# c0gent/hbbft

Measured on AMD Instinct MI355X. Metric: verified BLS sig shares/sec (whole node) + combine latency, N=64 f=21, higher is better.
Workload: dtype u32 limbs (Fp, 14x28-bit); 1 GPU; ThresholdSign share verification, BASELINE configs[1]; batch_per_gpu=65536, streams=2, documents_per_gpu=1024, n_nodes=64, f=21, pairing_impl=auto, parallelism=shard-by-batch x1

## Files before the change

hbbft_amd/csrc/k_pair.hip:

```cpp
#define HS_MULFN static __device__ __noinline__
#include "pair_side.hpp"

namespace hbs {

constexpr int EXP_TOP = 57;
constexpr uint64_t EXP_HIGH = hb::X_ABS >> EXP_TOP;
constexpr int EXP_HIGH_BITS = 64 - EXP_TOP;
constexpr int EXP_NPARK = __builtin_popcountll(hb::X_ABS) - __builtin_popcountll(EXP_HIGH) + 1;
static_assert((hb::X_ABS & 1) == 0 && (hb::X_ABS >> 63) == 1 && (EXP_HIGH & 1) == 1 && EXP_NPARK >= 1,
              "the base is no factor of f^|x|, and the power at bit EXP_TOP is the last one parked");
struct ExpPark {
  int32_t c[EXP_NPARK][4][NL];
  int32_t base[6][NL];
  int32_t pre[EXP_NPARK][NL];
};

HP_D void park_fp(int32_t (&d)[NL], const Fp& a) {
#pragma unroll
  for (int i = 0; i < NL; i++) d[i] = a.l[i];
}
HP_D Fp unpark_fp(const int32_t (&s)[NL]) {
  Fp r;
#pragma unroll
  for (int i = 0; i < NL; i++) r.l[i] = s[i];
  return r;
}
HP_D H12 unpark12(const int32_t (&s)[6][NL]) {
  return {{unpark_fp(s[0]), unpark_fp(s[1]), unpark_fp(s[2])}, {unpark_fp(s[3]), unpark_fp(s[4]), unpark_fp(s[5])}};
}

static __device__ __noinline__ void h_exp_gs(const ExpPark& pk, bool plus1, H12& out) {
  const uint64_t e = hb::X_ABS + (plus1 ? 1 : 0);
  H12 r = unpark12(pk.base);
#pragma unroll 1
  for (int k = 62; k >= 0; k--) {
    r = h12_cyclo_sqr(r);
    if ((e >> k) & 1) r = h12_mul<LanePair>(r, unpark12(pk.base));
  }
  out = r;
}

HP_D H12 h_exp_high(const H12& t) {
  H12 r = t;
#pragma unroll 1
  for (int k = EXP_HIGH_BITS - 2; k >= 0; k--) {
    r = h12_cyclo_sqr(r);
    if ((EXP_HIGH >> k) & 1) r = h12_mul<LanePair>(r, t);
  }
  return r;
}

static __device__ __noinline__ bool h_exp_tail(ExpPark& pk, bool plus1, H12& out) {
  Fp P;
#pragma unroll 1
  for (int j = 0; j < EXP_NPARK; j++) {
    const Fp d = hc_denom(unpark_fp(pk.c[j][0]));
    if (j == 0) P = d; else P = h_mul(P, d);
    park_fp(pk.pre[j], P);
  }
  if (h_is_zero(P)) return false;
  Fp I = fp_reduce(h_inv_vartime(P));
  H12 acc;
#pragma unroll 1
  for (int j = EXP_NPARK - 1; j >= (plus1 ? -1 : 0); j--) {
    H12 E;
    if (j >= 0) {
      const HC c = {unpark_fp(pk.c[j][0]), unpark_fp(pk.c[j][1]), unpark_fp(pk.c[j][2]), unpark_fp(pk.c[j][3])};
      Fp di = I;
      if (j > 0) {
        di = h_mul(I, unpark_fp(pk.pre[j - 1]));
        I = h_mul(I, hc_denom(c.a1));
      }
      E = hc_decompress(c, di);
    } else {
      E = unpark12(pk.base);
    }
    if (j == EXP_NPARK - 1) acc = h_exp_high(E); else acc = h12_mul<LanePair>(acc, E);
  }
  out = acc;
  return true;
}

template <bool PLUS1>
HP_D H12 h_exp_abs_x(const H12& base, ExpPark& pk) {
  park_fp(pk.base[0], base.c0.c0); park_fp(pk.base[1], base.c0.c1); park_fp(pk.base[2], base.c0.c2);
  park_fp(pk.base[3], base.c1.c0); park_fp(pk.base[4], base.c1.c1); park_fp(pk.base[5], base.c1.c2);
  HC c = hc_compress(base);
  int slot = 0;
#pragma unroll 1
  for (int k = 1; k <= EXP_TOP; k++) {
    c = hc_sqr(c);
    if ((hb::X_ABS >> k) & 1) {
      park_fp(pk.c[slot][0], c.a1); park_fp(pk.c[slot][1], c.a2);
      park_fp(pk.c[slot][2], c.a4); park_fp(pk.c[slot][3], c.a5);
      slot++;
    }
  }
  H12 r;
  if (!h_exp_tail(pk, PLUS1, r)) h_exp_gs(pk, PLUS1, r);
  return r;
}
struct ExpCompressed {
  ExpPark pk;
  HP_D H12 x(const H12& f) { return h12_conj(h_exp_abs_x<false>(f, pk)); }
  HP_D H12 xm1(const H12& f) { return h12_conj(h_exp_abs_x<true>(f, pk)); }
};

template <bool W1, bool W2, int GEN>
__global__ void __launch_bounds__(256, 2) k_pair_verify(PairArgs a) {
  extern __shared__ uint32_t stash_lds[];
  lane_verify<LanePair, ExpCompressed, W1, W2, GEN>(a, stash_lds);
}

}

namespace hbl {

struct PairKernels {
  static constexpr int LANES = hbs::LanePair::LANES;
  template <bool W1, bool W2, int GEN>
  static constexpr auto kernel = hbs::k_pair_verify<W1, W2, GEN>;
};

size_t pair_table_bytes(size_t nq) { return nq * (size_t)hbs::PAIR_STEPS * hbs::LINE_Q4 * 16; }

hipError_t pair_verify(hipStream_t s, int n, const PairSideDesc& d1, const PairSideDesc& d2, int flags,
                       uint8_t* verdict, uint32_t* value_out) {
  if (n <= 0) return hipSuccess;
  const int gen = pair_gen_mode(d1, d2);
  if (gen == 1) return lane_launch<PairKernels, 1>(s, n, d1, d2, flags, verdict, value_out);
  if (gen == 2) return lane_launch<PairKernels, 2>(s, n, d1, d2, flags, verdict, value_out);
  return lane_launch<PairKernels, 0>(s, n, d1, d2, flags, verdict, value_out);
}

}
```

hbbft_amd/csrc/pfp.hpp:

```cpp
#pragma once
#include "sfp.hpp"
#include "words.hpp"

#define HP_D __device__ __forceinline__
#define HP_L __attribute__((always_inline))

namespace hbs {

constexpr int DPP_SWAP = 0xB1;
constexpr int DPP_EVEN = 0xA0;
constexpr int DPP_ODD = 0xF5;

HP_D bool lp_even() { return (threadIdx.x & 1) == 0; }
template <int CTRL>
HP_D int32_t dpp(int32_t v) {
  return __builtin_amdgcn_mov_dpp(v, CTRL, 0xF, 0xF, true);
}
template <int CTRL>
HP_D Fp dpp_fp(const Fp& a) {
  Fp r;
#pragma unroll
  for (int i = 0; i < NL; i++) r.l[i] = dpp<CTRL>(a.l[i]);
  return r;
}

HS_MULFN Fp h_mul_l(HS_P14(x), HS_P14(y)) {
  const Fp a = {{HS_L14(x)}};
  const Fp b = {{HS_L14(y)}};
  const int32_t sm = lp_even() ? -1 : 0;
  int32_t Y[NL], W[NL], Z[NL];
#pragma unroll
  for (int i = 0; i < NL; i++) {
    Y[i] = dpp<DPP_EVEN>(b.l[i]);
    W[i] = dpp<DPP_ODD>(b.l[i]);
    Z[i] = (dpp<DPP_SWAP>(a.l[i]) ^ sm) - sm;
  }
  int32_t m[NL];
  int64_t acc = 0;
  Fp r;
#pragma unroll
  for (int k = 0; k < NL; k++) {
#pragma unroll
    for (int i = 0; i <= k; i++) {
      acc += (int64_t)a.l[i] * Y[k - i];
      acc += (int64_t)Z[i] * W[k - i];
    }
#pragma unroll
    for (int i = 0; i < k; i++) acc += (int64_t)m[i] * (int32_t)P_L[k - i];
    m[k] = mont_digit(acc);
    acc += (int64_t)m[k] * (int32_t)P_L[0];
    acc >>= 28;
  }
#pragma unroll
  for (int k = NL; k < 2 * NL - 1; k++) {
#pragma unroll
    for (int i = k - NL + 1; i < NL; i++) {
      acc += (int64_t)a.l[i] * Y[k - i];
      acc += (int64_t)Z[i] * W[k - i];
      acc += (int64_t)m[i] * (int32_t)P_L[k - i];
    }
    r.l[k - NL] = (int32_t)acc & MASK28;
    acc >>= 28;
  }
  r.l[NL - 1] = (int32_t)acc;
  return r;
}

HP_D Fp h_mul(const Fp& a, const Fp& b) { return h_mul_l(HS_E14(a), HS_E14(b)); }

HP_D Fp h_sqr(const Fp& a) {
  const bool ev = lp_even();
  const Fp pa = dpp_fp<DPP_SWAP>(a);
  Fp x, y;
#pragma unroll
  for (int i = 0; i < NL; i++) {
    x.l[i] = pa.l[i] + (ev ? a.l[i] : pa.l[i]);
    y.l[i] = a.l[i] - (ev ? pa.l[i] : 0);
  }
  return fp_mul(x, y);
}

HP_D Fp h_mul_xi(const Fp& a) {
  const int32_t sm = lp_even() ? -1 : 0;
  const Fp pa = dpp_fp<DPP_SWAP>(a);
  Fp r;
#pragma unroll
  for (int i = 0; i < NL; i++) r.l[i] = a.l[i] + ((pa.l[i] ^ sm) - sm);
  fp_norm(r);
  return r;
}
HP_D Fp h_conj(const Fp& a) {
  const Fp n = fp_neg(a);
  return lp_even() ? a : n;
}
HP_D Fp h_zero() { return fp_zero(); }
HP_D Fp h_one() { return lp_even() ? fp_one() : fp_zero(); }
HP_D Fp h_const(const uint32_t (&c0)[NL], const uint32_t (&c1)[NL]) {
  Fp r;
  const bool ev = lp_even();
#pragma unroll
  for (int i = 0; i < NL; i++) r.l[i] = (int32_t)(ev ? c0[i] : c1[i]);
  return r;
}
HP_D bool lp_both(bool v) { return (v ? 1 : 0) & dpp<DPP_SWAP>(v ? 1 : 0); }
HP_D bool h_is_zero(const Fp& a) { return lp_both(fp_is_zero(a)); }
template <int MODE = 0>
HP_D Fp h_inv_vartime(const Fp& a) {
  const Fp s = fp_sqr(a);
  const Fp n = fp_add(s, dpp_fp<DPP_SWAP>(s));
  uint32_t w[12], p[12], r[12];
  fp_to_words(n, w);
  uint32_t nz = 0;
#pragma unroll
  for (int i = 0; i < 12; i++) nz |= w[i];
  if (nz == 0) return fp_zero();
#pragma unroll
  for (int i = 0; i < 12; i++) p[i] = hb::PM2_W[i];
  p[0] += 2;
  hb::words_inv_vartime<12, MODE>(w, p, r);
  return h_conj(fp_mul(a, fp_from_words(r)));
}

template <int M, int K>
HP_D Fp fp_red_mk(const Fp& t, const Fp& a) {
  const int64_t top = (int64_t)t.l[NL - 1] * M + (int64_t)K * a.l[NL - 1];
  const int32_t q = (int32_t)((top * QINV) >> 32);
  Fp r;
  int64_t acc = 0;
#pragma unroll
  for (int i = 0; i < NL - 1; i++) {
    acc += (int64_t)t.l[i] * M + (int64_t)K * a.l[i] - (int64_t)q * (int32_t)P_L[i];
    r.l[i] = (int32_t)acc & MASK28;
    acc >>= 28;
  }
  r.l[NL - 1] = (int32_t)(acc + top - (int64_t)q * (int32_t)P_L[NL - 1]);
  return r;
}
HP_D Fp fp_red_l(const Fp& t) { return fp_red_mk<1, 0>(t, t); }
HP_D Fp h_add_xi_l(const Fp& s, const Fp& t) {
  const int32_t sm = lp_even() ? -1 : 0;
  const Fp pt = dpp_fp<DPP_SWAP>(t);
  Fp r;
#pragma unroll
  for (int i = 0; i < NL; i++) r.l[i] = s.l[i] + t.l[i] + ((pt.l[i] ^ sm) - sm);
  return r;
}
HP_D Fp fp_sub2l(const Fp& a, const Fp& b, const Fp& c) {
  Fp r;
#pragma unroll
  for (int i = 0; i < NL; i++) r.l[i] = a.l[i] - b.l[i] - c.l[i];
  return r;
}

HP_D Fp h_xi_l(const Fp& t) {
  const int32_t sm = lp_even() ? -1 : 0;
  const Fp pt = dpp_fp<DPP_SWAP>(t);
  Fp r;
#pragma unroll
  for (int i = 0; i < NL; i++) r.l[i] = t.l[i] + ((pt.l[i] ^ sm) - sm);
  return r;
}

struct H6 { Fp c0, c1, c2; };
struct H12 { H6 c0, c1; };

HP_D H6 h6_zero() { return {h_zero(), h_zero(), h_zero()}; }
HP_D H6 h6_one() { return {h_one(), h_zero(), h_zero()}; }
HP_D H6 h6_add(const H6& a, const H6& b) { return {fp_add(a.c0, b.c0), fp_add(a.c1, b.c1), fp_add(a.c2, b.c2)}; }
HP_D H6 h6_sub(const H6& a, const H6& b) { return {fp_sub(a.c0, b.c0), fp_sub(a.c1, b.c1), fp_sub(a.c2, b.c2)}; }
HP_D H6 h6_neg(const H6& a) { return {fp_neg(a.c0), fp_neg(a.c1), fp_neg(a.c2)}; }
HP_D H6 h6_red(const H6& a) { return {fp_reduce(a.c0), fp_reduce(a.c1), fp_reduce(a.c2)}; }
HP_D H6 h6_mul_v(const H6& a) { return {h_mul_xi(a.c2), a.c0, a.c1}; }

HP_D H6 h6_mul(const H6& a, const H6& b) {
  const Fp v1 = h_mul(a.c1, b.c1);
  const Fp v2 = h_mul(a.c2, b.c2);
  const Fp d0 = fp_sub2l(h_mul(fp_addl(a.c1, a.c2), fp_add(b.c1, b.c2)), v1, v2);
  const Fp v0 = h_mul(a.c0, b.c0);
  const Fp c0 = fp_red_l(h_add_xi_l(v0, d0));
  const Fp c1 = fp_red_l(h_add_xi_l(fp_sub2l(h_mul(fp_addl(a.c0, a.c1), fp_add(b.c0, b.c1)), v0, v1), v2));
  const Fp c2 = fp_red_l(fp_addl(fp_sub2l(h_mul(fp_addl(a.c0, a.c2), fp_add(b.c0, b.c2)), v0, v2), v1));
  return {c0, c1, c2};
}
HP_D H6 h6_inv(const H6& a) {
  const Fp c0 = fp_reduce(fp_sub(h_sqr(a.c0), h_mul_xi(h_mul(a.c1, a.c2))));
  const Fp c1 = fp_reduce(fp_sub(h_mul_xi(h_sqr(a.c2)), h_mul(a.c0, a.c1)));
  const Fp c2 = fp_reduce(fp_sub(h_sqr(a.c1), h_mul(a.c0, a.c2)));
  const Fp t = fp_reduce(fp_add(h_mul(a.c0, c0), h_mul_xi(fp_add(h_mul(a.c2, c1), h_mul(a.c1, c2)))));
  const Fp ti = fp_reduce(h_inv_vartime(t));
  return {h_mul(c0, ti), h_mul(c1, ti), h_mul(c2, ti)};
}

HP_D H12 h12_one() { return {h6_one(), h6_zero()}; }
HP_D H12 h12_conj(const H12& a) { return {a.c0, h6_neg(a.c1)}; }
HP_D H12 h12_red(const H12& a) { return {h6_red(a.c0), h6_red(a.c1)}; }
HP_D H12 h12_kcomb(const H6& t0, const H6& t1, const H6& s) {
  return {{fp_red_l(h_add_xi_l(t0.c0, t1.c2)), fp_red_l(fp_addl(t0.c1, t1.c0)), fp_red_l(fp_addl(t0.c2, t1.c1))},
          {fp_red_l(fp_sub2l(s.c0, t0.c0, t1.c0)), fp_red_l(fp_sub2l(s.c1, t0.c1, t1.c1)),
           fp_red_l(fp_sub2l(s.c2, t0.c2, t1.c2))}};
}

HP_D H6 h6_mul_12(const H6& x, const Fp& b1, const Fp& b2) {
  const Fp u = h_mul(x.c1, b1);
  const Fp w = h_mul(x.c2, b2);
  const Fp c0 = fp_red_l(h_xi_l(fp_sub2l(h_mul(fp_addl(x.c1, x.c2), fp_add(b1, b2)), u, w)));
  const Fp c1 = fp_red_l(h_add_xi_l(h_mul(x.c0, b1), w));
  const Fp c2 = fp_red_l(fp_addl(h_mul(x.c0, b2), u));
  return {c0, c1, c2};
}

HP_D const H6& h6_of(const H6& a) { return a; }
template <class F>
HP_D auto h6_of(const F& f) -> decltype(f()) { return f(); }

template <class G>
HP_D H12 h12_mul(const H12& a, const H12& b) {
  H6 t0, t1;
  G::mul6x2(a.c0, b.c0, a.c1, b.c1, t0, t1);
  const H6 s = G::mul6(h6_add(a.c0, a.c1), h6_add(b.c0, b.c1));
  return h12_kcomb(t0, t1, s);
}
template <class G>
HP_D H12 h12_sqr(const H12& a) {
  H6 t, s;
  G::mul6x2(a.c0, a.c1, [&]() HP_L { return h6_add(a.c0, a.c1); },
            [&]() HP_L { return h6_red(h6_add(a.c0, h6_mul_v(a.c1))); }, t, s);
  return {{fp_red_l(h_add_xi_l(fp_subl(s.c0, t.c0), fp_subl(fp_zero(), t.c2))), fp_red_l(fp_sub2l(s.c1, t.c1, t.c0)),
           fp_red_l(fp_sub2l(s.c2, t.c2, t.c1))},
          {fp_red_l(fp_addl(t.c0, t.c0)), fp_red_l(fp_addl(t.c1, t.c1)), fp_red_l(fp_addl(t.c2, t.c2))}};
}
template <class G>
HP_D H12 h12_mul_lines(const H12& f, const Fp& a0, const Fp& a1, const Fp& a4, const Fp& b0, const Fp& b1,
                       const Fp& b4) {
  H6 C0, t0, t1;
  Fp c11, c12;
  G::line_product(a0, a1, a4, b0, b1, b4, C0, c11, c12);
  G::mul6x2_12(f.c0, C0, f.c1, c11, c12, t0, t1);
  const H6 s = G::mul6(h6_add(f.c0, f.c1), {C0.c0, fp_add(C0.c1, c11), fp_add(C0.c2, c12)});
  return h12_kcomb(t0, t1, s);
}
template <class G>
HP_D H12 h12_inv(const H12& a) {
  H6 s0, s1, r0, r1;
  G::mul6x2(a.c0, a.c0, a.c1, a.c1, s0, s1);
  const H6 t = h6_red(h6_sub(h6_red(s0), h6_red(h6_mul_v(h6_red(s1)))));
  const H6 ti = h6_red(h6_inv(t));
  G::mul6x2(a.c0, ti, a.c1, ti, r0, r1);
  return h12_red({r0, h6_neg(r1)});
}

#define HP_FROB1(K) h_const(hb::FROB1_##K##_C0, hb::FROB1_##K##_C1)
HP_D H12 h12_frob1(const H12& f) {
  H12 r;
  r.c0.c0 = h_conj(f.c0.c0);
  r.c1.c0 = h_mul(h_conj(f.c1.c0), HP_FROB1(1));
  r.c0.c1 = h_mul(h_conj(f.c0.c1), HP_FROB1(2));
  r.c1.c1 = h_mul(h_conj(f.c1.c1), HP_FROB1(3));
  r.c0.c2 = h_mul(h_conj(f.c0.c2), HP_FROB1(4));
  r.c1.c2 = h_mul(h_conj(f.c1.c2), HP_FROB1(5));
  return h12_red(r);
}
HP_D H12 h12_frob2(const H12& f) {
  H12 r;
  r.c0.c0 = f.c0.c0;
  r.c1.c0 = fp_mul(f.c1.c0, fp_const(hb::FROB2_1_C0));
  r.c0.c1 = fp_mul(f.c0.c1, fp_const(hb::FROB2_2_C0));
  r.c1.c1 = fp_mul(f.c1.c1, fp_const(hb::FROB2_3_C0));
  r.c0.c2 = fp_mul(f.c0.c2, fp_const(hb::FROB2_4_C0));
  r.c1.c2 = fp_mul(f.c1.c2, fp_const(hb::FROB2_5_C0));
  return r;
}

HP_D H12 h12_cyclo_sqr(const H12& f) {
  const Fp& a0 = f.c0.c0; const Fp& a2 = f.c0.c1; const Fp& a4 = f.c0.c2;
  const Fp& a1 = f.c1.c0; const Fp& a3 = f.c1.c1; const Fp& a5 = f.c1.c2;
  H12 r;
  {
    const Fp s0 = h_sqr(a0), s3 = h_sqr(a3), s03 = h_sqr(fp_add(a0, a3));
    r.c0.c0 = fp_red_mk<3, -2>(h_add_xi_l(s0, s3), a0);
    r.c1.c1 = fp_red_mk<3, 2>(fp_sub2l(s03, s0, s3), a3);
  }
  {
    const Fp s1 = h_sqr(a1), s4 = h_sqr(a4), s14 = h_sqr(fp_add(a1, a4));
    r.c0.c1 = fp_red_mk<3, -2>(h_add_xi_l(s1, s4), a2);
    r.c1.c2 = fp_red_mk<3, 2>(fp_sub2l(s14, s1, s4), a5);
  }
  {
    const Fp s2 = h_sqr(a2), s5 = h_sqr(a5), s25 = h_sqr(fp_add(a2, a5));
    r.c0.c2 = fp_red_mk<3, -2>(h_add_xi_l(s2, s5), a4);
    r.c1.c0 = fp_red_mk<3, 2>(h_add_xi_l(fp_zero(), fp_sub2l(s25, s2, s5)), a1);
  }
  return r;
}

struct HC { Fp a1, a2, a4, a5; };

HP_D HC hc_compress(const H12& f) { return {f.c1.c0, f.c0.c1, f.c0.c2, f.c1.c2}; }
HP_D HC hc_sqr(const HC& c) {
  HC r;
  {
    const Fp s1 = h_sqr(c.a1), s4 = h_sqr(c.a4), s14 = h_sqr(fp_add(c.a1, c.a4));
    r.a2 = fp_red_mk<3, -2>(h_add_xi_l(s1, s4), c.a2);
    r.a5 = fp_red_mk<3, 2>(fp_sub2l(s14, s1, s4), c.a5);
  }
  {
    const Fp s2 = h_sqr(c.a2), s5 = h_sqr(c.a5), s25 = h_sqr(fp_add(c.a2, c.a5));
    r.a4 = fp_red_mk<3, -2>(h_add_xi_l(s2, s5), c.a4);
    r.a1 = fp_red_mk<3, 2>(h_add_xi_l(fp_zero(), fp_sub2l(s25, s2, s5)), c.a1);
  }
  return r;
}
HP_D Fp hc_denom(const Fp& a1) { return fp_lin(4, a1, 0, a1); }
HP_D H12 hc_decompress(const HC& c, const Fp& di) {
  const Fp s5 = h_sqr(c.a5), s2 = h_sqr(c.a2);
  Fp t = h_xi_l(s5);
#pragma unroll
  for (int i = 0; i < NL; i++) t.l[i] += 3 * s2.l[i];
  const Fp a3 = h_mul(fp_red_mk<1, -2>(t, c.a4), di);
  const Fp u = fp_addl(fp_lin(2, h_sqr(a3), -3, h_mul(c.a4, c.a2)), h_mul(c.a1, c.a5));
  const Fp a0 = fp_red_l(h_add_xi_l(h_one(), u));
  return {{a0, c.a2, c.a4}, {c.a1, a3, c.a5}};
}

HP_D bool h12_is_one(const H12& f) {
  bool ok = fp_is_zero(fp_sub(f.c0.c0, h_one()));
  ok = ok && fp_is_zero(f.c0.c1) && fp_is_zero(f.c0.c2);
  ok = ok && fp_is_zero(f.c1.c0) && fp_is_zero(f.c1.c1) && fp_is_zero(f.c1.c2);
  return lp_both(ok);
}

struct HJac { Fp x, y, z; };
struct HLine { Fp c0, c1, c4; };

struct HProj { Fp x, y, z; };

HP_D HLine h_dbl_step_h(HProj& T) {
  const Fp C = h_sqr(T.z);
  const Fp YZ = h_sqr(fp_add(T.y, T.z));
  const Fp B = h_sqr(T.y);
  const Fp H = fp_sub(fp_sub(YZ, B), C);
  const Fp E = fp_red_mk<12, 0>(h_xi_l(C), C);
  const Fp A = h_mul(T.x, T.y);
  const Fp S = h_sqr(T.x);
  HLine l;
  l.c0 = fp_red_mk<1, -1>(B, E);
  l.c1 = fp_lin(-3, S, 0, S);
  l.c4 = H;
  const Fp Bm = fp_lin(1, B, -3, E);
  const Fp Bp = fp_lin(1, B, 3, E);
  T.x = h_mul(fp_addl(A, A), Bm);
  const Fp EE = h_sqr(E);
  T.y = fp_red_mk<1, -12>(h_sqr(Bp), EE);
  const Fp BH = h_mul(fp_addl(B, B), H);
  T.z = fp_red_mk<2, 0>(BH, BH);
  return l;
}

HP_D HLine h_add_step_h(HProj& T, const Fp& xQ, const Fp& yQ) {
  const Fp th = fp_sub(T.y, h_mul(yQ, T.z));
  const Fp la = fp_sub(T.x, h_mul(xQ, T.z));
  HLine l;
  l.c0 = fp_reduce(fp_sub(h_mul(th, xQ), h_mul(la, yQ)));
  l.c1 = fp_neg(th);
  l.c4 = la;
  const Fp C = h_sqr(th);
  const Fp D = h_sqr(la);
  const Fp E = h_mul(la, D);
  const Fp F = h_mul(T.z, C);
  const Fp G = h_mul(T.x, D);
  const Fp H = fp_lin(1, fp_addl(E, F), -2, G);
  const Fp X3 = h_mul(la, H);
  T.y = fp_reduce(fp_sub(h_mul(th, fp_sub(G, H)), h_mul(E, T.y)));
  T.z = h_mul(T.z, E);
  T.x = X3;
  return l;
}

template <class PT>
struct SideStateT {
  Fp xP, yP;
  bool act;
  bool qinf;
  uint32_t q;
  PT T;
};

template <bool GEN, class ST>
HP_D Fp side_xP(const ST& st) { return GEN ? fp_const(hb::G1X_M) : st.xP; }
template <bool GEN, class ST>
HP_D Fp side_yP(const ST& st, bool negate) {
  return GEN ? (negate ? fp_neg(fp_const(hb::G1Y_M)) : fp_const(hb::G1Y_M)) : st.yP;
}

struct LanePair {
  static constexpr int LANES = 2;
  static HP_D bool leader() { return lp_even(); }
  static HP_D bool value_writer() { return true; }
  using Walk = HProj;
  static HP_D HLine dbl_step(HProj& T) { return h_dbl_step_h(T); }
  static HP_D HLine add_step(HProj& T, const Fp& xQ, const Fp& yQ) { return h_add_step_h(T, xQ, yQ); }

  static HP_D H6 mul6(const H6& a, const H6& b) { return h6_mul(a, b); }
  template <class A1, class B1>
  static HP_D void mul6x2(const H6& a0, const H6& b0, const A1& a1, const B1& b1, H6& r0, H6& r1) {
    r0 = h6_mul(a0, b0);
    r1 = h6_mul(h6_of(a1), h6_of(b1));
  }
  static HP_D void mul6x2_12(const H6& a0, const H6& b0, const H6& a1, const Fp& c1, const Fp& c2, H6& r0, H6& r1) {
    r0 = h6_mul(a0, b0);
    r1 = h6_mul_12(a1, c1, c2);
  }
  static HP_D void line_product(const Fp& a0, const Fp& a1, const Fp& a4, const Fp& b0, const Fp& b1, const Fp& b4,
                                H6& C0, Fp& c11, Fp& c12) {
    const Fp a0b0 = h_mul(a0, b0);
    const Fp a1b1 = h_mul(a1, b1);
    const Fp a4b4 = h_mul(a4, b4);
    c11 = fp_red_l(fp_sub2l(h_mul(fp_addl(a0, a4), fp_add(b0, b4)), a0b0, a4b4));
    c12 = fp_red_l(fp_sub2l(h_mul(fp_addl(a1, a4), fp_add(b1, b4)), a1b1, a4b4));
    C0 = {fp_red_l(h_add_xi_l(a0b0, a4b4)), fp_red_l(fp_sub2l(h_mul(fp_addl(a0, a1), fp_add(b0, b1)), a0b0, a1b1)),
          a1b1};
  }
  static HP_D H12 cyclo_sqr(const H12& f) { return h12_cyclo_sqr(f); }
  static HP_D H12 frob1(const H12& f) { return h12_frob1(f); }
  static HP_D H12 frob2(const H12& f) { return h12_frob2(f); }

  template <bool GEN, class ST>
  static HP_D HLine line_at_p(const HLine& l, const ST& st, bool negate) {
    HLine e;
    e.c0 = st.act ? l.c0 : h_one();
    e.c1 = st.act ? fp_mul(l.c1, side_xP<GEN>(st)) : fp_zero();
    e.c4 = st.act ? fp_mul(l.c4, side_yP<GEN>(st, negate)) : fp_zero();
    return e;
  }
  template <bool G1, bool G2, class RA, class RB, class ST>
  static HP_D void lines_at_p(const RA& raw_a, const RB& raw_b, const ST& A, const ST& B, bool neg2, HLine& la,
                              HLine& lb) {
    la = line_at_p<G1>(raw_a(), A, false);
    lb = line_at_p<G2>(raw_b(), B, neg2);
  }
};

HP_D void h_g2_load(const uint32_t* __restrict__ w, Fp& x, Fp& y) {
  const int o = lp_even() ? 0 : 12;
  x = fp_from_words(w + o);
  y = fp_from_words(w + 24 + o);
}
HP_D bool words_zero(const uint32_t* __restrict__ w, int n) {
  uint32_t o = 0;
  for (int k = 0; k < n; k++) o |= w[k];
  return o == 0;
}

}
```

hbbft_amd/csrc/words.hpp:

```cpp
#pragma once
#include <stdint.h>

#if defined(__HIPCC__) || defined(__HIP__)
#include <hip/hip_runtime.h>
#define HW_HD __host__ __device__ __forceinline__
#else
#define HW_HD inline
#endif

namespace hb {

template <int N>
HW_HD bool words_is_one(const uint32_t* x) {
  uint32_t o = x[0] ^ 1u;
  for (int i = 1; i < N; i++) o |= x[i];
  return o == 0;
}
template <int N>
HW_HD void words_shr1(uint32_t* x, uint32_t top) {
  for (int i = 0; i < N - 1; i++) x[i] = (x[i] >> 1) | (x[i + 1] << 31);
  x[N - 1] = (x[N - 1] >> 1) | (top << 31);
}
template <int N>
HW_HD uint32_t words_add(uint32_t* x, const uint32_t* y) {
  uint64_t c = 0;
  for (int i = 0; i < N; i++) {
    c += (uint64_t)x[i] + y[i];
    x[i] = (uint32_t)c;
    c >>= 32;
  }
  return (uint32_t)c;
}
template <int N>
HW_HD uint32_t words_sub(uint32_t* x, const uint32_t* y) {
  uint64_t br = 0;
  for (int i = 0; i < N; i++) {
    const uint64_t d = (uint64_t)x[i] - y[i] - br;
    x[i] = (uint32_t)d;
    br = (d >> 63) & 1;
  }
  return (uint32_t)br;
}
template <int N>
HW_HD bool words_geq(const uint32_t* x, const uint32_t* y) {
  for (int i = N - 1; i >= 0; i--)
    if (x[i] != y[i]) return x[i] > y[i];
  return true;
}
template <int N>
HW_HD int words_bitlen(const uint32_t* x) {
  int len = 0;
#pragma unroll
  for (int i = 0; i < N; i++)
    if (x[i]) len = 32 * i + 32 - __builtin_clz(x[i]);
  return len;
}
template <int N>
HW_HD uint64_t words_bits64(const uint32_t* x, int s) {
  const int w = s >> 5, sh = s & 31;
  uint32_t lo = 0, mid = 0, hi = 0;
#pragma unroll
  for (int i = 0; i < N; i++) {
    lo = (i == w) ? x[i] : lo;
    mid = (i == w + 1) ? x[i] : mid;
    hi = (i == w + 2) ? x[i] : hi;
  }
  const uint64_t v = (uint64_t)lo | ((uint64_t)mid << 32);
  return sh ? (v >> sh) | ((uint64_t)hi << (64 - sh)) : v;
}
template <int N>
HW_HD void words_lincomb_shr31(const uint32_t* x, int64_t fx, const uint32_t* y, int64_t fy, uint32_t* out) {
  uint32_t t[N + 2];
  int64_t c = 0;
#pragma unroll
  for (int i = 0; i < N; i++) {
    const int64_t p1 = (int64_t)x[i] * fx, p2 = (int64_t)y[i] * fy;
    const int64_t sw = (int64_t)(uint32_t)p1 + (int64_t)(uint32_t)p2 + c;
    t[i] = (uint32_t)sw;
    c = (sw >> 32) + (p1 >> 32) + (p2 >> 32);
  }
  t[N] = (uint32_t)c;
  t[N + 1] = (uint32_t)(c >> 32);
#pragma unroll
  for (int i = 0; i <= N; i++) out[i] = (t[i] >> 31) | (t[i + 1] << 1);
}
template <int N>
HW_HD bool words_neg_if(uint32_t* x, bool neg) {
  if (!neg) return false;
  uint64_t c = 1;
#pragma unroll
  for (int i = 0; i < N; i++) {
    c += (uint64_t)(uint32_t)~x[i];
    x[i] = (uint32_t)c;
    c >>= 32;
  }
  return true;
}

template <int N>
HW_HD void words_lin_mont31(const uint32_t* x, int64_t fx, const uint32_t* y, int64_t fy, const uint32_t* mod,
                            uint32_t minv, uint32_t* out) {
  const uint32_t t0 = (uint32_t)((uint64_t)x[0] * (uint64_t)fx + (uint64_t)y[0] * (uint64_t)fy);
  const uint64_t q = (uint64_t)((t0 * minv) & 0x7fffffffu);
  uint32_t t[N + 2];
  int64_t c = 0;
#pragma unroll
  for (int i = 0; i <= N; i++) {
    const int64_t xi = i < N ? (int64_t)x[i] : (int64_t)(int32_t)x[N];
    const int64_t yi = i < N ? (int64_t)y[i] : (int64_t)(int32_t)y[N];
    const int64_t p1 = xi * fx, p2 = yi * fy;
    const uint64_t p3 = i < N ? q * mod[i] : 0;
    const int64_t sw = (int64_t)(uint32_t)p1 + (int64_t)(uint32_t)p2 + (int64_t)(uint32_t)p3 + c;
    t[i] = (uint32_t)sw;
    c = (sw >> 32) + (p1 >> 32) + (p2 >> 32) + (int64_t)(p3 >> 32);
  }
  t[N + 1] = (uint32_t)c;
#pragma unroll
  for (int i = 0; i <= N; i++) out[i] = (t[i] >> 31) | (t[i + 1] << 1);
}

constexpr int INV_BATCH = 1, INV_LAZY = 2;
template <int N, int MODE = 0>
HW_HD void words_inv_vartime(const uint32_t* y, const uint32_t* mod, uint32_t* out) {
  constexpr bool BATCH = (MODE & INV_BATCH) != 0, LAZY = (MODE & INV_LAZY) != 0;
  uint32_t a[N + 1], b[N + 1], u[N + 1], v[N + 1];
#pragma unroll
  for (int i = 0; i < N; i++) {
    a[i] = y[i];
    b[i] = mod[i];
    u[i] = 0;
    v[i] = 0;
  }
  a[N] = b[N] = u[N] = v[N] = 0;
  u[0] = 1;
  uint32_t inv = mod[0];
  for (int k = 0; k < 5; k++) inv *= 2u - mod[0] * inv;
  const uint32_t minv = 0u - inv;
  const int rounds = (2 * words_bitlen<N>(mod) - 1 + 30) / 31;
  for (int r = 0; r < rounds; r++) {
    int n;
    if (LAZY) {
      uint32_t o[N];
#pragma unroll
      for (int i = 0; i < N; i++) o[i] = a[i] | b[i];
      n = words_bitlen<N>(o);
    } else {
      n = words_bitlen<N>(a);
      const int nb = words_bitlen<N>(b);
      if (nb > n) n = nb;
    }
    if (n < 64) n = 64;
    uint64_t ab = ((uint64_t)a[0] & 0x7fffffffu) | (words_bits64<N>(a, n - 33) << 31);
    uint64_t bb = ((uint64_t)b[0] & 0x7fffffffu) | (words_bits64<N>(b, n - 33) << 31);
    int64_t f0 = 1, g0 = 0, f1 = 0, g1 = 1;
    if (BATCH) {
      int j = 0;
      while (true) {
        const int tz = ab ? __builtin_ctzll(ab) : 64;
        const int z = tz < 31 - j ? tz : 31 - j;
        ab >>= z;
        f1 <<= z;
        g1 <<= z;
        j += z;
        if (j >= 31) break;
        if (ab < bb) {
          const uint64_t t = ab;
          ab = bb;
          bb = t;
          int64_t q = f0;
          f0 = f1;
          f1 = q;
          q = g0;
          g0 = g1;
          g1 = q;
        }
        ab = (ab - bb) >> 1;
        f0 -= f1;
        g0 -= g1;
        f1 *= 2;
        g1 *= 2;
        if (++j >= 31) break;
      }
    }
    for (int j = 0; j < (BATCH ? 0 : 31); j++) {
      if (ab & 1) {
        if (ab < bb) {
          const uint64_t t = ab;
          ab = bb;
          bb = t;
          int64_t q = f0;
          f0 = f1;
          f1 = q;
          q = g0;
          g0 = g1;
          g1 = q;
        }
        ab = (ab - bb) >> 1;
        f0 -= f1;
        g0 -= g1;
      } else {
        ab >>= 1;
      }
      f1 *= 2;
      g1 *= 2;
    }
    uint32_t na[N + 1], nbw[N + 1];
    words_lincomb_shr31<N>(a, f0, b, g0, na);
    words_lincomb_shr31<N>(a, f1, b, g1, nbw);
    if (words_neg_if<N + 1>(na, (int32_t)na[N] < 0)) {
      f0 = -f0;
      g0 = -g0;
    }
    if (words_neg_if<N + 1>(nbw, (int32_t)nbw[N] < 0)) {
      f1 = -f1;
      g1 = -g1;
    }
#pragma unroll
    for (int i = 0; i <= N; i++) {
      a[i] = na[i];
      b[i] = nbw[i];
    }
    if (LAZY) {
      uint32_t nu0[N + 1], nv0[N + 1];
      words_lin_mont31<N>(u, f0, v, g0, mod, minv, nu0);
      words_lin_mont31<N>(u, f1, v, g1, mod, minv, nv0);
#pragma unroll
      for (int i = 0; i <= N; i++) {
        u[i] = nu0[i];
        v[i] = nv0[i];
      }
      continue;
    }
    uint32_t nu[2][N + 1];
#pragma unroll
    for (int side = 0; side < 2; side++) {
      const int64_t fu = side ? f1 : f0, fv = side ? g1 : g0;
      uint32_t t[N + 2];
      int64_t c = 0;
#pragma unroll
      for (int i = 0; i < N; i++) {
        const int64_t p1 = (int64_t)u[i] * fu, p2 = (int64_t)v[i] * fv;
        const int64_t sw = (int64_t)(uint32_t)p1 + (int64_t)(uint32_t)p2 + c;
        t[i] = (uint32_t)sw;
        c = (sw >> 32) + (p1 >> 32) + (p2 >> 32);
      }
      t[N] = (uint32_t)c;
      t[N + 1] = (uint32_t)(c >> 32);
      const uint64_t q = (uint64_t)((t[0] * minv) & 0x7fffffffu);
      uint64_t cc = 0;
#pragma unroll
      for (int i = 0; i < N; i++) {
        cc += (uint64_t)t[i] + q * mod[i];
        t[i] = (uint32_t)cc;
        cc >>= 32;
      }
#pragma unroll
      for (int i = N; i < N + 2; i++) {
        cc += (uint64_t)t[i];
        t[i] = (uint32_t)cc;
        cc >>= 32;
      }
      uint32_t w[N + 1];
#pragma unroll
      for (int i = 0; i <= N; i++) w[i] = (t[i] >> 31) | (t[i + 1] << 1);
      for (int k = 0; k < 3 && (int32_t)w[N] < 0; k++) {
        uint64_t ac = 0;
#pragma unroll
        for (int i = 0; i < N; i++) {
          ac += (uint64_t)w[i] + mod[i];
          w[i] = (uint32_t)ac;
          ac >>= 32;
        }
        w[N] += (uint32_t)ac;
      }
      for (int k = 0; k < 3 && (w[N] != 0 || words_geq<N>(w, mod)); k++) {
        const uint32_t br = words_sub<N>(w, mod);
        w[N] -= br;
      }
#pragma unroll
      for (int i = 0; i <= N; i++) nu[side][i] = w[i];
    }
#pragma unroll
    for (int i = 0; i <= N; i++) {
      u[i] = nu[0][i];
      v[i] = nu[1][i];
    }
  }
  bool one = b[N] == 0 && words_is_one<N>(b);
  if (LAZY && one) {
    while ((int32_t)v[N] < 0) {
      const uint32_t c = words_add<N>(v, mod);
      v[N] += c;
    }
    while (v[N] != 0 || words_geq<N>(v, mod)) {
      const uint32_t br = words_sub<N>(v, mod);
      v[N] -= br;
    }
  }
#pragma unroll
  for (int i = 0; i < N; i++) out[i] = one ? v[i] : 0u;
}

}
```

Measured before the change: 3.604 million shares/s.

## Add constant-round lane-pair split field inversion for pairing exponentiation

Adds a fixed-round (uniform) binary GCD inversion with branch-free divsteps and signed-magnitude matrix application. It also adds a variant that splits each inversion's a/b and u/v updates across the two lanes of a pair, exchanging data through DPP swaps. The pairing kernel's exponent tail now uses the paired uniform inversion by default (mode 12), while h6_inv uses HP_INV_MODE, which resolves to 12 in this translation unit. The aim is to remove the divergence of the variable-time inversion, where lanes loop different iteration counts, and to halve the per-lane work. In exchange it always runs the worst-case round count and adds cross-lane traffic.

```diff
diff --git a/hbbft_amd/csrc/k_pair.hip b/hbbft_amd/csrc/k_pair.hip
--- a/hbbft_amd/csrc/k_pair.hip
+++ b/hbbft_amd/csrc/k_pair.hip
@@ -1,4 +1,7 @@
 #define HS_MULFN static __device__ __noinline__
+#ifndef HP_INV_MODE
+#define HP_INV_MODE 12
+#endif
 #include "pair_side.hpp"
 
 namespace hbs {
@@ -59,7 +62,7 @@
     park_fp(pk.pre[j], P);
   }
   if (h_is_zero(P)) return false;
-  Fp I = fp_reduce(h_inv_vartime(P));
+  Fp I = fp_reduce(h_inv_vartime<HP_INV_MODE>(P));
   H12 acc;
 #pragma unroll 1
   for (int j = EXP_NPARK - 1; j >= (plus1 ? -1 : 0); j--) {
diff --git a/hbbft_amd/csrc/pfp.hpp b/hbbft_amd/csrc/pfp.hpp
--- a/hbbft_amd/csrc/pfp.hpp
+++ b/hbbft_amd/csrc/pfp.hpp
@@ -1,6 +1,10 @@
 #pragma once
 #include "sfp.hpp"
 #include "words.hpp"
+
+#ifndef HP_INV_MODE
+#define HP_INV_MODE 0
+#endif
 
 #define HP_D __device__ __forceinline__
 #define HP_L __attribute__((always_inline))
@@ -104,6 +108,101 @@
 }
 HP_D bool lp_both(bool v) { return (v ? 1 : 0) & dpp<DPP_SWAP>(v ? 1 : 0); }
 HP_D bool h_is_zero(const Fp& a) { return lp_both(fp_is_zero(a)); }
+constexpr int INV_PAIR = 8;
+template <int N>
+HP_D void lp_inv_uniform(const uint32_t* y, const uint32_t* mod, uint32_t* out) {
+  static_assert(N <= 15, "words_reduce_32m");
+  const bool ev = lp_even();
+  uint32_t mine[N], other[N], co[N + 1];
+#pragma unroll
+  for (int i = 0; i < N; i++) {
+    mine[i] = ev ? y[i] : mod[i];
+    other[i] = ev ? mod[i] : y[i];
+    co[i] = 0;
+  }
+  co[N] = 0;
+  co[0] = ev ? 1u : 0u;
+  uint32_t inv = mod[0];
+  for (int k = 0; k < 5; k++) inv *= 2u - mod[0] * inv;
+  const uint32_t minv = 0u - inv;
+  const int rounds = (2 * hb::words_bitlen<N>(mod) - 1 + 30) / 31;
+#pragma unroll 1
+  for (int r = 0; r < rounds; r++) {
+    const uint64_t am = hb::words_approx<N>(mine, hb::words_len2<N>(mine, other));
+    const uint64_t ao = (uint64_t)(uint32_t)dpp<DPP_SWAP>((int32_t)(uint32_t)am) |
+                        ((uint64_t)(uint32_t)dpp<DPP_SWAP>((int32_t)(uint32_t)(am >> 32)) << 32);
+    uint64_t ab = ev ? am : ao, bb = ev ? ao : am;
+    uint32_t c0 = ev ? 1u : 0u, c1 = ev ? 0u : 1u;
+#pragma unroll 1
+    for (int j = 0; j < 31; j++) {
+      uint32_t odd;
+      bool sw;
+      hb::words_divstep_ab(ab, bb, odd, sw);
+      hb::words_divstep_col(c0, c1, odd, sw);
+    }
+    uint32_t km, ks, sm, ss;
+    hb::words_fac_split(ev ? c0 : c1, km, ks);
+    hb::words_fac_split(ev ? c1 : c0, sm, ss);
+    {
+      uint32_t t[N + 2], k[N + 2], row[N + 1];
+      hb::words_mul_sm<N, false>(mine, sm, ss, t);
+#pragma unroll
+      for (int i = 0; i < N + 2; i++) t[i] = (uint32_t)dpp<DPP_SWAP>((int32_t)t[i]);
+      hb::words_mul_sm<N, false>(mine, km, ks, k);
+      uint64_t c = 0;
+#pragma unroll
+      for (int i = 0; i < N + 2; i++) {
+        c += (uint64_t)k[i] + t[i];
+        t[i] = (uint32_t)c;
+        c >>= 32;
+      }
+#pragma unroll
+      for (int i = 0; i <= N; i++) row[i] = (t[i] >> 31) | (t[i + 1] << 1);
+      const uint32_t fl = hb::words_abs<N + 1>(row);
+      ks ^= fl;
+      ss ^= (uint32_t)dpp<DPP_SWAP>((int32_t)fl);
+#pragma unroll
+      for (int i = 0; i < N; i++) {
+        mine[i] = row[i];
+        other[i] = (uint32_t)dpp<DPP_SWAP>((int32_t)row[i]);
+      }
+    }
+    {
+      uint32_t t[N + 2], w[N + 2];
+      hb::words_mul_sm<N, true>(co, sm, ss, t);
+#pragma unroll
+      for (int i = 0; i < N + 2; i++) t[i] = (uint32_t)dpp<DPP_SWAP>((int32_t)t[i]);
+      const uint32_t xe = 0u - (co[N] >> 31);
+      const uint32_t k0 = km & ks;
+      const uint64_t q = (uint64_t)(((k0 + (co[0] ^ ks) * km + t[0]) * minv) & 0x7fffffffu);
+      uint64_t c = k0;
+#pragma unroll
+      for (int i = 0; i < N + 2; i++) {
+        const uint32_t xi = (i <= N ? co[i] : xe) ^ ks;
+        c += (uint64_t)xi * km;
+        if (i < N) c += q * mod[i];
+        c += t[i];
+        w[i] = (uint32_t)c;
+        c >>= 32;
+      }
+#pragma unroll
+      for (int i = 0; i <= N; i++) co[i] = (w[i] >> 31) | (w[i + 1] << 1);
+    }
+  }
+  const uint32_t mine_one = hb::words_is_one<N>(mine) ? 1u : 0u;
+  const uint32_t part_one = (uint32_t)dpp<DPP_SWAP>((int32_t)mine_one);
+  const bool one = (ev ? part_one : mine_one) != 0;
+  uint32_t v[N + 1];
+#pragma unroll
+  for (int i = 0; i <= N; i++) {
+    const uint32_t pv = (uint32_t)dpp<DPP_SWAP>((int32_t)co[i]);
+    v[i] = ev ? pv : co[i];
+  }
+  hb::words_reduce_32m<N>(v, mod);
+#pragma unroll
+  for (int i = 0; i < N; i++) out[i] = one ? v[i] : 0u;
+}
+
 template <int MODE = 0>
 HP_D Fp h_inv_vartime(const Fp& a) {
   const Fp s = fp_sqr(a);
@@ -117,7 +216,10 @@
 #pragma unroll
   for (int i = 0; i < 12; i++) p[i] = hb::PM2_W[i];
   p[0] += 2;
-  hb::words_inv_vartime<12, MODE>(w, p, r);
+  if ((MODE & INV_PAIR) != 0)
+    lp_inv_uniform<12>(w, p, r);
+  else
+    hb::words_inv_vartime<12, MODE>(w, p, r);
   return h_conj(fp_mul(a, fp_from_words(r)));
 }
 
@@ -187,7 +289,7 @@
   const Fp c1 = fp_reduce(fp_sub(h_mul_xi(h_sqr(a.c2)), h_mul(a.c0, a.c1)));
   const Fp c2 = fp_reduce(fp_sub(h_sqr(a.c1), h_mul(a.c0, a.c2)));
   const Fp t = fp_reduce(fp_add(h_mul(a.c0, c0), h_mul_xi(fp_add(h_mul(a.c2, c1), h_mul(a.c1, c2)))));
-  const Fp ti = fp_reduce(h_inv_vartime(t));
+  const Fp ti = fp_reduce(h_inv_vartime<HP_INV_MODE>(t));
   return {h_mul(c0, ti), h_mul(c1, ti), h_mul(c2, ti)};
 }
 
diff --git a/hbbft_amd/csrc/words.hpp b/hbbft_amd/csrc/words.hpp
--- a/hbbft_amd/csrc/words.hpp
+++ b/hbbft_amd/csrc/words.hpp
@@ -119,9 +119,191 @@
   for (int i = 0; i <= N; i++) out[i] = (t[i] >> 31) | (t[i + 1] << 1);
 }
 
-constexpr int INV_BATCH = 1, INV_LAZY = 2;
+constexpr int INV_BATCH = 1, INV_LAZY = 2, INV_UNIFORM = 4;
+
+HW_HD void words_fac_split(uint32_t f, uint32_t& mag, uint32_t& sgn) {
+  const uint32_t s = 0u - (f >> 31);
+  mag = (f ^ s) - s;
+  sgn = mag == 0x80000000u ? 0u : s;
+}
+template <int N, bool SIGNED>
+HW_HD void words_lin_sm31(const uint32_t* x, uint32_t fm, uint32_t fs, const uint32_t* y, uint32_t gm, uint32_t gs,
+                          const uint32_t* mod, uint32_t minv, uint32_t* out) {
+  const uint32_t xe = SIGNED ? 0u - (x[N] >> 31) : 0u, ye = SIGNED ? 0u - (y[N] >> 31) : 0u;
+  const uint32_t c0 = (fm & fs) + (gm & gs);
+  uint64_t q = 0;
+  if (SIGNED) q = (uint64_t)(((c0 + (x[0] ^ fs) * fm + (y[0] ^ gs) * gm) * minv) & 0x7fffffffu);
+  uint32_t t[N + 2];
+  uint64_t c = c0;
+#pragma unroll
+  for (int i = 0; i < N + 2; i++) {
+    const uint32_t xi = (i < N + (SIGNED ? 1 : 0) ? x[i] : xe) ^ fs;
+    const uint32_t yi = (i < N + (SIGNED ? 1 : 0) ? y[i] : ye) ^ gs;
+    c += (uint64_t)xi * fm + (uint64_t)yi * gm;
+    if (SIGNED && i < N) c += q * mod[i];
+    t[i] = (uint32_t)c;
+    c >>= 32;
+  }
+#pragma unroll
+  for (int i = 0; i <= N; i++) out[i] = (t[i] >> 31) | (t[i + 1] << 1);
+}
+template <int N, bool SIGNED>
+HW_HD void words_mul_sm(const uint32_t* x, uint32_t m, uint32_t s, uint32_t* t) {
+  const uint32_t xe = SIGNED ? 0u - (x[N] >> 31) : 0u;
+  uint64_t c = m & s;
+#pragma unroll
+  for (int i = 0; i < N + 2; i++) {
+    const uint32_t xi = (i < N + (SIGNED ? 1 : 0) ? x[i] : xe) ^ s;
+    c += (uint64_t)xi * m;
+    t[i] = (uint32_t)c;
+    c >>= 32;
+  }
+}
+template <int N>
+HW_HD uint32_t words_abs(uint32_t* x) {
+  const uint32_t s = 0u - (x[N - 1] >> 31);
+  uint64_t c = s & 1u;
+#pragma unroll
+  for (int i = 0; i < N; i++) {
+    c += (uint64_t)(x[i] ^ s);
+    x[i] = (uint32_t)c;
+    c >>= 32;
+  }
+  return s;
+}
+template <int N>
+HW_HD int words_len2(const uint32_t* a, const uint32_t* b) {
+  int n = 64;
+#pragma unroll
+  for (int i = 2; i < N; i++) {
+    const uint32_t o = a[i] | b[i];
+    n = o ? 32 * i + 32 - __builtin_clz(o) : n;
+  }
+  return n;
+}
+template <int N>
+HW_HD uint64_t words_approx(const uint32_t* x, int n) {
+  const int s = n - 33, w = s >> 5, sh = s & 31;
+  uint32_t lo = 0, mid = 0, hi = 0;
+#pragma unroll
+  for (int i = 0; i < N; i++) {
+    lo = (i == w) ? x[i] : lo;
+    mid = (i == w + 1) ? x[i] : mid;
+    hi = (i == w + 2) ? x[i] : hi;
+  }
+  const uint64_t t = (((uint64_t)lo | ((uint64_t)mid << 32)) >> sh) | ((((uint64_t)hi) << 1) << (63 - sh));
+  return ((uint64_t)x[0] & 0x7fffffffu) | (t << 31);
+}
+HW_HD void words_divstep_ab(uint64_t& ab, uint64_t& bb, uint32_t& odd, bool& sw) {
+  odd = 0u - ((uint32_t)ab & 1u);
+  const uint64_t bm = bb & (((uint64_t)odd << 32) | odd);
+  sw = ab < bm;
+  const uint64_t d = ab - bm, nd = bm - ab;
+  bb = sw ? ab : bb;
+  ab = (sw ? nd : d) >> 1;
+}
+HW_HD void words_divstep_col(uint32_t& c0, uint32_t& c1, uint32_t odd, bool sw) {
+  const uint32_t x0 = sw ? c1 : c0, x1 = sw ? c0 : c1;
+  c0 = x0 - (x1 & odd);
+  c1 = x1 << 1;
+}
+template <int N>
+HW_HD void words_reduce_32m(uint32_t* v, const uint32_t* mod) {
+  uint64_t c = 0;
+#pragma unroll
+  for (int i = 0; i <= N; i++) {
+    const uint32_t mk = (i < N ? mod[i] << 5 : 0u) | (i > 0 ? mod[i - 1] >> 27 : 0u);
+    c += (uint64_t)v[i] + mk;
+    v[i] = (uint32_t)c;
+    c >>= 32;
+  }
+#pragma unroll
+  for (int k = 5; k >= 0; k--) {
+    uint32_t t[N + 1];
+    uint64_t br = 0;
+#pragma unroll
+    for (int i = 0; i <= N; i++) {
+      const uint32_t mk = (i < N ? mod[i] << k : 0u) | (i > 0 ? (mod[i - 1] >> 1) >> (31 - k) : 0u);
+      const uint64_t d = (uint64_t)v[i] - mk - br;
+      t[i] = (uint32_t)d;
+      br = (d >> 63) & 1;
+    }
+#pragma unroll
+    for (int i = 0; i <= N; i++) v[i] = br ? v[i] : t[i];
+  }
+}
+
+template <int N>
+HW_HD void words_inv_uniform(const uint32_t* y, const uint32_t* mod, uint32_t* out) {
+  static_assert(N <= 15, "rounds <= 31: |v| < 32 m, and 64 m fits N+1 words");
+  uint32_t a[N + 1], b[N + 1], u[N + 1], v[N + 1];
+#pragma unroll
+  for (int i = 0; i < N; i++) {
+    a[i] = y[i];
+    b[i] = mod[i];
+    u[i] = 0;
+    v[i] = 0;
+  }
+  a[N] = b[N] = u[N] = v[N] = 0;
+  u[0] = 1;
+  uint32_t inv = mod[0];
+  for (int k = 0; k < 5; k++) inv *= 2u - mod[0] * inv;
+  const uint32_t minv = 0u - inv;
+  const int rounds = (2 * words_bitlen<N>(mod) - 1 + 30) / 31;
+#pragma unroll 1
+  for (int r = 0; r < rounds; r++) {
+    const int n = words_len2<N>(a, b);
+    uint64_t ab = words_approx<N>(a, n), bb = words_approx<N>(b, n);
+    uint32_t f0 = 1, g0 = 0, f1 = 0, g1 = 1;
+#if defined(__HIP_DEVICE_COMPILE__)
+#pragma unroll 1
+#endif
+    for (int j = 0; j < 31; j++) {
+      uint32_t odd;
+      bool sw;
+      words_divstep_ab(ab, bb, odd, sw);
+      words_divstep_col(f0, f1, odd, sw);
+      words_divstep_col(g0, g1, odd, sw);
+    }
+    uint32_t m0, s0, m1, s1, m2, s2, m3, s3;
+    words_fac_split(f0, m0, s0);
+    words_fac_split(g0, m1, s1);
+    words_fac_split(f1, m2, s2);
+    words_fac_split(g1, m3, s3);
+    uint32_t na[N + 1], nb[N + 1];
+    words_lin_sm31<N, false>(a, m0, s0, b, m1, s1, mod, minv, na);
+    words_lin_sm31<N, false>(a, m2, s2, b, m3, s3, mod, minv, nb);
+    const uint32_t fa = words_abs<N + 1>(na), fb = words_abs<N + 1>(nb);
+    s0 ^= fa;
+    s1 ^= fa;
+    s2 ^= fb;
+    s3 ^= fb;
+#pragma unroll
+    for (int i = 0; i <= N; i++) {
+      a[i] = na[i];
+      b[i] = nb[i];
+    }
+    uint32_t nu[N + 1], nv[N + 1];
+    words_lin_sm31<N, true>(u, m0, s0, v, m1, s1, mod, minv, nu);
+    words_lin_sm31<N, true>(u, m2, s2, v, m3, s3, mod, minv, nv);
+#pragma unroll
+    for (int i = 0; i <= N; i++) {
+      u[i] = nu[i];
+      v[i] = nv[i];
+    }
+  }
+  const bool one = b[N] == 0 && words_is_one<N>(b);
+  words_reduce_32m<N>(v, mod);
+#pragma unroll
+  for (int i = 0; i < N; i++) out[i] = one ? v[i] : 0u;
+}
+
 template <int N, int MODE = 0>
 HW_HD void words_inv_vartime(const uint32_t* y, const uint32_t* mod, uint32_t* out) {
+  if ((MODE & INV_UNIFORM) != 0) {
+    words_inv_uniform<N>(y, mod, out);
+    return;
+  }
   constexpr bool BATCH = (MODE & INV_BATCH) != 0, LAZY = (MODE & INV_LAZY) != 0;
   uint32_t a[N + 1], b[N + 1], u[N + 1], v[N + 1];
 #pragma unroll
```

Measured after the change: 3.690 million shares/s, median of 6. 1.02x the previous value.
